# wuer5/OMGSR

Measured on AMD Instinct MI355X. Metric: SR images/sec, higher is better.
Workload: dtype fp16; 1 GPU; OMGSR-S 256->1024, batch=4/GPU, accurate tier (fp32 stream, fp16 MFMA operands + split corrections), tiled VAE 256/64; global_batch=4, latent_tile=64, tile_overlap=32, world_size=1, parallelism=dp1, weights=seeded random, SD2.1-base shapes

## Files before the change

### include/omgsr_hip.h

```cpp
#ifndef OMGSR_HIP_H
#define OMGSR_HIP_H

#include <stdint.h>

#ifdef __cplusplus
extern "C" {
#endif

#define OMGSR_E_BADARG (-1)
#define OMGSR_E_SHAPE (-2)
#define OMGSR_E_ARCH (-3)

#define OMGSR_ACT_NONE 0
#define OMGSR_ACT_SILU 1
#define OMGSR_ACT_GELU_TANH 2
#define OMGSR_ACT_GEGLU 3

#define OMGSR_OUT_BF16 0
#define OMGSR_OUT_F32 1

#define OMGSR_LAYOUT_NHWC 0
#define OMGSR_LAYOUT_T 1

#define OMGSR_EL_16 0
// ... 46 lines not shown
    int32_t mx_scale_w1, mx_scale_a1, mx_scale_w2, mx_scale_a2;
    int32_t out_mx;
    int32_t group_tiles;
    uint32_t* overflow_flag;
    const float* gn_scale_shift;
    int32_t gn_nimg;
    int32_t gn_act;
    int32_t in_el;
    int32_t mx_fmt;
    int32_t mxf8;
    int32_t mxf8_reserved;
    const uint8_t* in_scale;
    const uint8_t* w_scale;
} omgsr_igemm_args;
int32_t omgsr_igemm_gn_fusable(const omgsr_igemm_args* a);
int32_t omgsr_igemm_out_mx6_ok(const omgsr_igemm_args* a);
int omgsr_groupnorm_scale_shift(const float* mean, const float* rstd, const float* gamma, const float* beta, float* out, int32_t nimg, int32_t C,
                                int32_t G, void* stream);
int omgsr_igemm(const omgsr_igemm_args* a, void* stream);
int32_t omgsr_conv_mxfp8_ok(const omgsr_igemm_args* a);
int omgsr_conv_mxfp8(const omgsr_igemm_args* a, void* stream);
int32_t omgsr_conv_mxfp8_multi_ok(const omgsr_igemm_args* args, int32_t count);
int omgsr_conv_mxfp8_multi(const omgsr_igemm_args* args, int32_t count, void* stream);
int omgsr_igemm_multi_plan(omgsr_igemm_args* args, int32_t count);
int omgsr_igemm_multi(const omgsr_igemm_args* args, int32_t count, void* stream);
int omgsr_set_batch_invariant(int on);
int64_t omgsr_igemm_workspace_bytes(const omgsr_igemm_args* a);
int32_t omgsr_igemm_gn_slots(const omgsr_igemm_args* a);
int32_t omgsr_igemm_gn_entries(const omgsr_igemm_args* a);

int omgsr_groupnorm_nchunk(int64_t HW);
int omgsr_groupnorm_stats(const void* x, float* partial, float* mean, float* rstd, float* var_out,
                          int32_t N, int64_t HW, int32_t C, int32_t G, float eps, int32_t x_el, void* stream);
int omgsr_groupnorm_finalize(const float* partial, float* mean, float* rstd, float* var_out, int32_t N,
                             int32_t nslot, int32_t G, int32_t entries, double count, float eps, void* stream);
int omgsr_groupnorm_partial(const void* x, float* partial, int32_t N, int64_t HW, int32_t C, int32_t G, int32_t x_el, void* stream);
#define OMGSR_GN_MAX_GROUPS 8
typedef struct omgsr_gn_merge_args {
    const float* partial[OMGSR_GN_MAX_GROUPS];
    double count[OMGSR_GN_MAX_GROUPS];
    float weight[OMGSR_GN_MAX_GROUPS];
    int32_t tiles[OMGSR_GN_MAX_GROUPS];
    int32_t nslot[OMGSR_GN_MAX_GROUPS];
    int32_t entries[OMGSR_GN_MAX_GROUPS];
    int32_t ngroups;
} omgsr_gn_merge_args;
// ... 122 lines not shown
```

### omgsr_amd/_lib.py

```python
from __future__ import annotations

import ctypes as C
import os

import torch

from .build import lib_path

ABI_VERSION = 22


class OmgsrError(RuntimeError):
    pass


class IgemmArgs(C.Structure):
    _fields_ = [
        ("in_", C.c_void_p), ("weight", C.c_void_p), ("bias", C.c_void_p), ("gate", C.c_void_p),
        ("residual", C.c_void_p), ("out", C.c_void_p),
        ("N", C.c_int32), ("H", C.c_int32), ("W", C.c_int32), ("Cin", C.c_int32),
        ("Cout", C.c_int32), ("Cout_pad", C.c_int32), ("K_pad", C.c_int32),
        ("R", C.c_int32), ("S", C.c_int32), ("stride", C.c_int32), ("pad_top", C.c_int32),
        ("pad_left", C.c_int32), ("upsample", C.c_int32),
        ("Ho", C.c_int32), ("Wo", C.c_int32),
# ... 45 lines not shown

_P, _I, _L, _F = C.c_void_p, C.c_int32, C.c_int64, C.c_float

SIGNATURES = {
    "omgsr_abi_version": (C.c_int, []),
    "omgsr_check_device": (C.c_int, []),
    "omgsr_set_compute_dtype": (C.c_int, [C.c_int]),
    "omgsr_get_compute_dtype": (C.c_int, []),
    "omgsr_error_string": (C.c_char_p, [C.c_int]),
    "omgsr_igemm": (C.c_int, [C.POINTER(IgemmArgs), _P]),
    "omgsr_igemm_multi_plan": (C.c_int, [C.POINTER(IgemmArgs), _I]),
    "omgsr_igemm_multi": (C.c_int, [C.POINTER(IgemmArgs), _I, _P]),
    "omgsr_set_batch_invariant": (C.c_int, [C.c_int]),
    "omgsr_set_attention_defer_max": (C.c_int, [C.c_float]),
    "omgsr_igemm_workspace_bytes": (C.c_int64, [C.POINTER(IgemmArgs)]),
    "omgsr_igemm_gn_slots": (C.c_int32, [C.POINTER(IgemmArgs)]),
    "omgsr_igemm_gn_entries": (C.c_int32, [C.POINTER(IgemmArgs)]),
    "omgsr_igemm_gn_fusable": (C.c_int32, [C.POINTER(IgemmArgs)]),
    "omgsr_igemm_out_mx6_ok": (C.c_int32, [C.POINTER(IgemmArgs)]),
    "omgsr_conv_mxfp8_ok": (C.c_int32, [C.POINTER(IgemmArgs)]),
    "omgsr_conv_mxfp8": (C.c_int, [C.POINTER(IgemmArgs), _P]),
    "omgsr_conv_mxfp8_multi_ok": (C.c_int32, [C.POINTER(IgemmArgs), _I]),
    "omgsr_conv_mxfp8_multi": (C.c_int, [C.POINTER(IgemmArgs), _I, _P]),
    "omgsr_groupnorm_apply_mxfp8": (C.c_int, [_P, _P, _P, _P, _P, _P, _P, _I, _L, _I, _I, _I, _I, _I, _P]),
    "omgsr_groupnorm_apply_mxfp8_multi": (C.c_int, [C.POINTER(GnApplyGroup), _I, _P, _P, _P, _P, _I, _I, _I, _I, _I, _P]),
    "omgsr_groupnorm_scale_shift": (C.c_int, [_P, _P, _P, _P, _P, _I, _I, _I, _P]),
    "omgsr_groupnorm_finalize": (C.c_int, [_P, _P, _P, _P, _I, _I, _I, _I, C.c_double, _F, _P]),
    "omgsr_groupnorm_partial": (C.c_int, [_P, _P, _I, _L, _I, _I, _I, _P]),
    "omgsr_groupnorm_finalize_merged": (C.c_int, [C.POINTER(GnMergeArgs), _P, _P, _P, _I, _I, _F, _P]),
    "omgsr_groupnorm_apply_shared": (C.c_int, [_P, _P, _P, _P, _P, _P, _I, _L, _I, _I, _I, _I, _I, _I, _P, _I, _P, _P]),
    "omgsr_groupnorm_apply_multi": (C.c_int, [C.POINTER(GnApplyGroup), _I, _P, _P, _P, _P, _I, _I, _I, _I, _I, _I, _I, _P, _P]),
    "omgsr_groupnorm_finalize2": (C.c_int, [_P, _I, _I, _P, _I, _I, _P, _P, _P, _I, _I, C.c_double, _F, _P]),
    "omgsr_groupnorm_apply2": (C.c_int, [_P, _P, _I, _P, _P, _P, _P, _P, _I, _L, _I, _I, _I, _I, _P, _I, _P, _P]),
    "omgsr_image_to_model_input": (C.c_int, [_P, _P, _I, _I, _I, _I, _P]),
    "omgsr_colorfix_workspace_bytes": (C.c_int64, [_I, _I, _I, _I]),
    "omgsr_colorfix": (C.c_int, [_P, _I, _P, _P, _P, _I, _I, _I, _I, _I, _P]),
    "omgsr_groupnorm_nchunk": (C.c_int, [_L]),
    "omgsr_groupnorm_stats": (C.c_int, [_P, _P, _P, _P, _P, _I, _L, _I, _I, _F, _I, _P]),
    "omgsr_groupnorm_apply": (C.c_int, [_P, _P, _P, _P, _P, _P, _I, _L, _I, _I, _I, _I, _I, _P, _I, _P, _P]),
    "omgsr_layernorm": (C.c_int, [_P, _P, _P, _P, _L, _I, _F, _I, _I, _P]),
    "omgsr_resize_nearest_exact_nhwc": (C.c_int, [_P, _P, _I, _I, _I, _I, _I, _I, _F, _F, _I, _P]),
    "omgsr_transpose_split": (C.c_int, [_P, _P, _I, _I, _I, _L, _P]),
    "omgsr_to_operand": (C.c_int, [_P, _P, _L, _I, _I, _P, _P]),
    "omgsr_quantize_mxfp8": (C.c_int, [_P, _I, _L, _I, _L, _P, _P, _P]),
    "omgsr_attention": (C.c_int, [C.POINTER(AttnArgs), _P]),
    "omgsr_softmax_rows": (C.c_int, [_P, _P, _L, _I, _I, _P]),
# ... 53 lines not shown
```

### omgsr_amd/build.py

```python
from __future__ import annotations

import hashlib
import os
import shutil
import subprocess
import sys

HERE = os.path.dirname(os.path.abspath(__file__))
CSRC = os.path.join(HERE, "csrc")
LIBDIR = os.path.join(HERE, "lib")
LIBNAME = "libomgsr_hip.so"
SOURCES = ["igemm.hip", "igemm_dma.hip", "igemm_p8.hip", "igemm_gmx.hip", "igemm_halo.hip", "igemm_halo_f16.hip", "igemm_halo_multi.hip", "igemm_halo_mx.hip", "igemm_halo_mx6.hip", "igemm_halo_mx6_flat.hip", "igemm_halo_out6.hip", "igemm_halo_flat.hip", "igemm_halo_gn.hip", "attention.hip", "norm.hip", "elementwise.hip", "colorfix.hip", "preprocess.hip", "mfma_peak.hip", "gemm_mxfp8.hip", "attention_mxfp8.hip", "attention_d512.hip", "conv_mxfp8.hip"]
ARCH = "gfx950"


def lib_path() -> str:
    return os.path.join(LIBDIR, LIBNAME)


def _source_digest() -> str:
    h = hashlib.sha256()
    names = sorted(os.listdir(CSRC)) + [os.path.join("..", "..", "include", "omgsr_hip.h")]
    for n in names:
        p = os.path.join(CSRC, n)
        if os.path.isfile(p):
            h.update(n.encode())
            with open(p, "rb") as f:
                h.update(f.read())
    return h.hexdigest()


def build_library(force: bool = False, verbose: bool = False) -> str:
    hipcc = shutil.which("hipcc") or "/opt/rocm/bin/hipcc"
    os.makedirs(LIBDIR, exist_ok=True)
    out = lib_path()
# ... 127 lines not shown
```

### omgsr_amd/nn.py

```python
from __future__ import annotations

import dataclasses
from typing import Optional

import torch
import torch.nn as nn

from . import ops


def _key(*tensors) -> tuple:
    return ops.mode_key() + tuple((t.data_ptr(), t._version, str(t.device), t.dtype, tuple(t.shape)) if torch.is_tensor(t) else t for t in tensors)


_CACHE_EPOCH = 0


def cache_epoch() -> int:
    return _CACHE_EPOCH


def bump_cache_epoch() -> None:
    global _CACHE_EPOCH
    _CACHE_EPOCH += 1
# ... 79 lines not shown

    def packed_mxfp8(self) -> ops.PackedWeight:
        k = _key(self.weight, self.bias, "mxfp8-conv")
        if getattr(self, "_pk8_key", None) != k:
            bump_cache_epoch()
            _log_rebuild(self._drop_packed_mxfp8)
            self._pk8 = ops.pack_conv_weight_mxfp8(self.weight, self.bias)
            self._pk8_key = k
        return self._pk8

    def _drop_packed_mxfp8(self) -> None:
        self._pk8, self._pk8_key = None, None
        bump_cache_epoch()

    def packed(self) -> ops.PackedWeight:
        sp, wsp, ph = self.in_split(), self.in_wsplit(), self.phase_upsample
        return self._packed(lambda: ops.pack_conv_weight(self.weight, self.bias, cout_multiple=8, split=sp, w_split=wsp, upsample_phases=ph),
                            self.weight, self.bias, sp, wsp, ph)

    def nhwc(self, x, *, pad=None, upsample=False, act=ops.ACT_NONE, residual=None, bias_override=None, stride=None, gn_groups=0,
             out_dtype=ops.OUT_STREAM, out_split=1, gn=None):
        pw = self.packed()
        if bias_override is not None:
            pw = dataclasses.replace(pw, bias=bias_override)
        p = self.padding[0] if pad is None else pad
        if out_dtype == ops.OUT_STREAM and self.out_inner16 and ops.precise():
            out_dtype = ops.OUT_BF16
        fp8_pack = self.packed_mxfp8 if (self.fp8 and gn is not None and bias_override is None) else None
        return ops.conv2d(x, pw, stride=stride or self.stride[0], pad=p, upsample=upsample, act=act, residual=residual,
                          gn_groups=gn_groups, out_dtype=out_dtype, out_split=out_split, gn=gn, fp8_pack=fp8_pack)

    def nhwc_multi(self, xs, *, pad=None, upsample=False, act=ops.ACT_NONE, residuals=None, stride=None, gn_groups=0,
                   out_dtype=ops.OUT_STREAM, out_split=1, gn=None, fp8=False):
        pw = self.packed()
        p = self.padding[0] if pad is None else pad
        if out_dtype == ops.OUT_STREAM and self.out_inner16 and ops.precise():
            out_dtype = ops.OUT_BF16
        fp8_pack = self.packed_mxfp8 if (fp8 and self.fp8 and gn is not None) else None
        return ops.conv2d_multi(list(xs), pw, stride=stride or self.stride[0], pad=p, upsample=upsample, act=act, residuals=residuals,
                                gn_groups=gn_groups, out_dtype=out_dtype, out_split=out_split, gn=gn, fp8_pack=fp8_pack)

    def forward(self, x):
        y = self.nhwc(ops.nchw_to_nhwc(x.contiguous(), ops._round_up(self.in_channels, 8)))
        return ops.nhwc_to_nchw(y, channels=self.out_channels,
                                dtype=ops.io_dtype(x))


# ... 85 lines not shown
```

### omgsr_amd/ops.py

```python
from __future__ import annotations

import ctypes as C
import os
from dataclasses import dataclass
from typing import Optional

import torch

from . import _lib
from ._lib import AttnArgs, IgemmArgs, check

ACT_NONE, ACT_SILU, ACT_GELU_TANH, ACT_GEGLU = 0, 1, 2, 3
OUT_STREAM, OUT_BF16, OUT_F32 = -1, 0, 1
LAYOUT_NHWC, LAYOUT_T = 0, 1
EL_16, EL_F32, EL_SPLIT, EL_MX, EL_MX6, EL_MXFP8 = 0, 1, 2, 3, 4, 5
MX_LO_SHIFT = 11


def _el_of_split(split: int) -> int:
    return {1: EL_16, 2: EL_SPLIT, 3: EL_MX, 4: EL_MX6}[split]


_ACT = torch.bfloat16
_PRECISE = False
# ... 86 lines not shown
_mx_saturated = False


def mx_saturation_seen(reset: bool = True) -> bool:
    global _mx_saturated
    for t in _ovf_words.values():
        if int(t.item()) & 2:
            _mx_saturated = True
            if reset:
                t.bitwise_and_(1)
    seen = _mx_saturated
    if reset:
        _mx_saturated = False
    return seen


_BATCH_INVARIANT = False


def set_batch_invariant(on: bool) -> None:
    global _BATCH_INVARIANT
    check(_lib.load().omgsr_set_batch_invariant(int(bool(on))), "omgsr_set_batch_invariant")
    _BATCH_INVARIANT = bool(on)


STAGE_NONE, STAGE_ENCODE, STAGE_DENOISE, STAGE_DECODE = 0, 1, 2, 3


def timing_stage(stage: int) -> None:
    _lib.load().omgsr_timing_stage(stage)


def compute_dtype_name() -> str:
    return "fp32" if _PRECISE else ("bf16" if _ACT == torch.bfloat16 else "fp16")


def io_dtype(x: torch.Tensor) -> torch.dtype:
    return torch.float32 if x.dtype == torch.float32 else _ACT


def _el(t: torch.Tensor, name: str) -> int:
    if not t.is_cuda:
        raise _lib.OmgsrError(f"{name}: tensor is on {t.device}; the OMGSR HIP path runs on an MI355X only")
    if not t.is_contiguous():
        raise ValueError(f"{name}: must be contiguous")
    if t.dtype == torch.float32:
# ... 33 lines not shown
        ws = torch.empty(need // 4, device=device, dtype=torch.float32)
        a.workspace = ws.data_ptr()
    check(lib.omgsr_igemm(C.byref(a), _stream()), what)



@dataclass
class PackedWeight:
    w: torch.Tensor
    bias: Optional[torch.Tensor]
    cout: int
    cin: int
    R: int
    S: int
    geglu: bool = False
    w_cm: Optional[torch.Tensor] = None
    split: int = 1
    mx: Optional[tuple] = None
    mx_fmt: int = 0
    w_split: int = 1
    in_ld: int = 0
    w_ph: Optional[torch.Tensor] = None
    w_scale: Optional[torch.Tensor] = None

    @property
    def fp8(self) -> bool:
        return self.w_scale is not None

    @property
    def cout_pad(self) -> int:
        return self.w.shape[0]

    @property
    def k_pad(self) -> int:
        return self.w.shape[1]

    @property
    def row_channels(self) -> int:
        return self.in_ld or self.cin


def _segments(w: torch.Tensor, split: int, w_split: int) -> torch.Tensor:
    w_hi = w.to(act_dtype()).float()
    segs = [w_hi] * split
    if w_split == 2:
        segs.append((w - w_hi).to(act_dtype()).float())
# ... 66 lines not shown
    b = None if bias is None else bias.detach().to(device=dev, dtype=torch.float32).contiguous()
    if fmt == 6:
        return PackedWeight(out, b, cout, kslots, R, S, w_cm=w_cm, split=4, w_split=1, in_ld=kslots, w_ph=w_ph, mx=(cin // 32, 127, 127, 127, 127), mx_fmt=6)
    return PackedWeight(out, b, cout, kslots, R, S, w_cm=w_cm, split=3, w_split=1, in_ld=kslots, w_ph=w_ph,
                        mx=(cin // 32, 127 - s1, 127 - MX_LO_SHIFT, 127 - s2, 127))


def _phase_kernels(w: torch.Tensor) -> torch.Tensor:
    rows = {0: ([0], [1, 2]), 1: ([0, 1], [2])}
    w64 = w.double()
    out = []
    for a in (0, 1):
        for b in (0, 1):
            k = torch.zeros((w.shape[0], 2, 2, w.shape[3]), dtype=torch.float64, device=w.device)
            for dy, rs in enumerate(rows[a]):
                for dx, ss in enumerate(rows[b]):
                    for r in rs:
                        for s_ in ss:
                            k[:, dy, dx] += w64[:, r, s_]
            out.append(k.float())
    return torch.stack(out, 0)


def pack_conv_weight(weight: torch.Tensor, bias: Optional[torch.Tensor], device=None, cout_multiple: int = 1,
                     split: int = 1, w_split: int = 1, upsample_phases: bool = False) -> PackedWeight:
    cout, cin, R, S = weight.shape
    dev = device or weight.device
    if cout % cout_multiple:
        extra = _round_up(cout, cout_multiple) - cout
        weight = torch.cat([weight.detach().to(dev), torch.zeros((extra, cin, R, S), device=dev, dtype=weight.dtype)], dim=0)
        if bias is not None:
            bias = torch.cat([bias.detach().to(dev), torch.zeros(extra, device=dev, dtype=bias.dtype)], dim=0)
        cout += extra
    cin8 = _round_up(cin, 8)
    w = _note_weight_range(weight.detach().to(device=dev, dtype=torch.float32)).permute(0, 2, 3, 1)
    if cin8 != cin:
        w = torch.nn.functional.pad(w, (0, cin8 - cin))
    if split in (3, 4):
        if cin8 != cin:
            raise ValueError("the mixed-precision (MX) form needs Cin % 64 == 0")
        return _pack_mx(w, bias if bias is None else bias.detach().to(dev), cout, cin, R, S, dev, upsample_phases, fmt=6 if split == 4 else 8)
    if split not in (1, 2) or w_split not in (1, 2):
        raise ValueError("split / w_split must be 1 or 2")
    if w_split == 2 and bool(torch.equal(w.to(act_dtype()).float(), w)):
        ph_exact = True
        if upsample_phases and R == 3 and S == 3:
            ph0 = _phase_kernels(w)
            ph_exact = bool(torch.equal(ph0.to(act_dtype()).float(), ph0))
        if ph_exact:
            w_split = 1
    in_ld = cin8 * split
    w_raw = w
    w = _segments(w, split, w_split)
    cin8 = w.shape[-1]
    w = w.reshape(cout, R * S * cin8)
    k_pad = _round_up(w.shape[1], 32)
    cout_pad = _round_up(cout, 256 if cout >= 256 else 128)
    out = torch.zeros(cout_pad, k_pad, device=dev, dtype=act_dtype())
    out[:cout, : w.shape[1]] = w.to(act_dtype())
    b = None if bias is None else bias.detach().to(device=dev, dtype=torch.float32).contiguous()
    w_cm = None
    if R == 3 and S == 3 and cin8 % 32 == 0:
        w_cm = out.view(cout_pad, 9, cin8 // 32, 32).permute(2, 1, 0, 3).contiguous()
    w_ph = None
    if upsample_phases and w_cm is not None and in_ld % 32 == 0:
        ph = _segments(_phase_kernels(w_raw), split, w_split).reshape(4, cout, 4 * cin8)
        full = torch.zeros((4, cout_pad, 4 * cin8), device=dev, dtype=act_dtype())
        full[:, :cout] = ph.to(act_dtype())
        w_ph = full.view(4, cout_pad, 4, cin8 // 32, 32).permute(0, 3, 2, 1, 4).contiguous()
    return PackedWeight(out, b, cout, cin8, R, S, w_cm=w_cm, split=split, w_split=w_split, in_ld=in_ld, w_ph=w_ph)


def pack_linear_weight(weight: torch.Tensor, bias: Optional[torch.Tensor], device=None, split: int = 1, w_split: int = 1) -> PackedWeight:
    return pack_conv_weight(weight[:, :, None, None], bias, device, split=split, w_split=w_split)


def pack_geglu_weight(weight: torch.Tensor, bias: Optional[torch.Tensor], device=None, split: int = 1, w_split: int = 1) -> PackedWeight:
    two_inner, cin = weight.shape
    inner = two_inner // 2
    if inner % 32:
        raise ValueError("GEGLU inner dim must be a multiple of 32")
    a, g = weight[:inner], weight[inner:]
    w = torch.stack([a.reshape(inner // 32, 32, cin), g.reshape(inner // 32, 32, cin)], dim=1).reshape(two_inner, cin)
    pw = pack_linear_weight(w, None, device, split=split, w_split=w_split)
    if bias is not None:
        ba, bg = bias[:inner], bias[inner:]
        b = torch.stack([ba.reshape(-1, 32), bg.reshape(-1, 32)], dim=1).reshape(two_inner)
        pw.bias = b.detach().to(device=pw.w.device, dtype=torch.float32).contiguous()
    pw.cout = inner
    pw.geglu = True
    return pw


# ... 201 lines not shown

    def apply(self, x: torch.Tensor, split: int = 1) -> torch.Tensor:
        if split == 5:
            return group_norm_apply_mxfp8(x, self.mean, self.rstd, self.gamma, self.beta, self.groups, self.act)
        if self.mean.shape[0] != x.shape[0]:
            return group_norm_apply_shared(x, self.mean, self.rstd, self.gamma, self.beta, self.groups, self.act, split=split)
        return group_norm_apply(x, self.mean, self.rstd, self.gamma, self.beta, self.groups, self.act, split=split)


def _gn_candidate(x: torch.Tensor, pw: PackedWeight) -> bool:
    return x.dtype == _ACT and pw.split == 1 and pw.w_split == 1 and pw.mx is None and pw.R == 3 and pw.S == 3


def _gn_fusable(a: IgemmArgs, gn: "GnSpec") -> bool:
    return gn.act == ACT_SILU and bool(_lib.load().omgsr_igemm_gn_fusable(C.byref(a)))


def _attach_gn(a: IgemmArgs, gn: "GnSpec", channels: int) -> torch.Tensor:
    t = gn.table(channels)
    a.gn_scale_shift, a.gn_nimg, a.gn_act, a.in_el = t.data_ptr(), t.shape[0], gn.act, EL_16
    return t


def conv2d(x: torch.Tensor, pw: PackedWeight, *, stride: int = 1, pad: tuple[int, int, int, int] | int = 1,
           upsample: bool = False, act: int = ACT_NONE, residual: Optional[torch.Tensor] = None,
           gate: Optional[torch.Tensor] = None, out_dtype: int = OUT_STREAM, alpha: float = 1.0,
           out: Optional[torch.Tensor] = None, gn_groups: int = 0, out_split: int = 1, sample_rows: int = 0,
           gn: Optional["GnSpec"] = None, fp8_pack=None) -> torch.Tensor:
    a = IgemmArgs()
    if gn is not None and not _gn_candidate(x, pw):
        x, gn = gn.apply(x, pw.split), None
    x, out = _conv_args(a, x, pw, stride, pad, upsample, act, residual, gate, out_dtype, alpha, out, out_split, sample_rows)
    if fp8_pack is not None and gn is not None and out_split == 1 and _lib.load().omgsr_conv_mxfp8_ok(C.byref(a)):
        return _conv2d_mxfp8(a, gn.apply(x, 5), fp8_pack(), out, gn_groups)
    if out_split == 4 and not _lib.load().omgsr_igemm_out_mx6_ok(C.byref(a)):
        return to_operand(conv2d(x, pw, stride=stride, pad=pad, upsample=upsample, act=act, residual=residual, gate=gate, out_dtype=OUT_STREAM,
                                 alpha=alpha, sample_rows=sample_rows, gn=gn), 4)
    keep = None
    if gn is not None:
        a.in_el = EL_16
        if _gn_fusable(a, gn):
            keep = _attach_gn(a, gn, x.shape[-1])
        else:
            x = gn.apply(x, pw.split)
            a.in_ = x.data_ptr()
    partial = _conv_gn(a, gn_groups, out_split, x.device)
    _igemm(a, x.device, "omgsr_igemm(conv2d)")
    del keep
    if partial is not None:
        out._omgsr_gn = (partial, gn_groups, out.data_ptr(), out._version)
    return out

# ... 74 lines not shown
        a = arr[i]
        out = _out_tensor((N, H, W), pw8.cout, out_dtype, 1, xq.codes.device)
        residual = None if residuals is None else residuals[i]
        if residual is not None and tuple(residual.shape) != (N, H, W, pw8.cout):
            raise ValueError(f"residual shape {tuple(residual.shape)} != output {(N, H, W, pw8.cout)}")
        _fill_out(a, out, 1, residual, pw8.cout)
        a.N, a.H, a.W, a.Cin, a.Cout = N, H, W, Cin, pw8.cout
        a.R, a.S, a.stride, a.pad_top, a.pad_left, a.upsample = 3, 3, 1, 1, 1, 0
        a.Ho, a.Wo, a.act, a.out_layout = H, W, act, LAYOUT_NHWC
        a.batch, a.alpha, a.sample_rows = 1, 1.0, H * W
        a.overflow_flag = None
        outs.append(out)
    return _conv2d_mxfp8_multi(arr, n, xqs, pw8, outs, gn_groups)


def conv2d_multi(xs, pw: PackedWeight, *, stride: int = 1, pad: tuple[int, int, int, int] | int = 1, upsample: bool = False,
                 act: int = ACT_NONE, residuals=None, out_dtype: int = OUT_STREAM, gn_groups: int = 0, out_split: int = 1,
                 gn: Optional["GnSpec"] = None, fp8_pack=None):
    n = len(xs)
    if n == 1:
        return [conv2d(xs[0], pw, stride=stride, pad=pad, upsample=upsample, act=act, residual=None if residuals is None else residuals[0],
                       out_dtype=out_dtype, gn_groups=gn_groups, out_split=out_split, gn=gn, fp8_pack=fp8_pack)]
    lib = _lib.load()
    if gn is not None and not all(_gn_candidate(x, pw) for x in xs):
        xs, gn = [gn.apply(x, pw.split) for x in xs], None
    arr = (IgemmArgs * n)()
    keep, outs = [], []
    for i in range(n):
        x, out = _conv_args(arr[i], xs[i], pw, stride, pad, upsample, act, None if residuals is None else residuals[i], None, out_dtype, 1.0,
                            None, out_split, 0)
        keep.append(x)
        outs.append(out)
        if gn is not None:
            arr[i].in_el = EL_16
    if fp8_pack is not None and gn is not None and out_split == 1 and lib.omgsr_conv_mxfp8_multi_ok(arr, n):
        xqs = []
        for k in range(0, n, _lib.GN_MAX_GROUPS):
            xqs += group_norm_apply_mxfp8_multi(keep[k:k + _lib.GN_MAX_GROUPS], gn.mean, gn.rstd, gn.gamma, gn.beta, gn.groups, gn.act)
        return _conv2d_mxfp8_multi(arr, n, xqs, fp8_pack(), outs, gn_groups)
    check(lib.omgsr_igemm_multi_plan(arr, n), "omgsr_igemm_multi_plan")
    if out_split == 4 and not all(lib.omgsr_igemm_out_mx6_ok(C.byref(arr[i])) for i in range(n)):
        ys = conv2d_multi(keep, pw, stride=stride, pad=pad, upsample=upsample, act=act, residuals=residuals, out_dtype=OUT_STREAM, gn=gn)
        return [to_operand(y, 4) for y in ys]
    if gn is not None:
        if all(_gn_fusable(arr[i], gn) for i in range(n)):
            for i in range(n):
# ... 793 lines not shown
```

### omgsr_amd/pipelines/vaehook.py

```python
from __future__ import annotations

import math
from typing import Dict, List, Tuple

import torch

from .. import ops


def get_best_tile_size(lowerbound: int, upperbound: int) -> int:
    divider = 32
    while divider >= 2:
        rem = lowerbound % divider
        if rem == 0:
            return lowerbound
        cand = lowerbound - rem + divider
        if cand <= upperbound:
            return cand
        divider //= 2
    return lowerbound


def split_tiles(h: int, w: int, tile_size: int, pad: int, is_decoder: bool) -> Tuple[List[List[int]], List[List[int]]]:
    nh = max(math.ceil((h - 2 * pad) / tile_size), 1)
# ... 71 lines not shown
            return self.net.nhwc(x)
        return self.vae_tile_forward(x)

    def _run(self, seq, groups: Dict[tuple, torch.Tensor], counts: Dict[tuple, int], N: int, fixed=None, record=None):
        res: Dict[tuple, list] = {k: [] for k in groups}
        gi = 0
        pending = None
        for op in seq:
            kind = op[0]
            if kind == "gn":
                norm, act = op[1], op[2]
                G = norm.num_groups
                if fixed is not None:
                    mean, var = fixed[gi]
                    rstd = torch.rsqrt(var + 1e-6)
                else:
                    keys = list(groups)
                    mean, rstd, var = ops.group_norm_stats_merged([groups[k] for k in keys], [counts[k] for k in keys], N, G, 1e-6)
                if record is not None:
                    record.append((mean, var))
                gi += 1
                first = next(iter(groups.values()))
                is_conv3 = getattr(op[3], "kernel_size", None) == (3, 3)
                if is_conv3 and first.dtype != torch.float32:
                    pending = norm.spec_stats(mean, rstd, act)
                    if op[4] is not None:
                        for k in groups:
                            res[k].append(op[4].nhwc(groups[k], pad=0))
                    continue
                keys = list(groups)
                if op[4] is not None:
                    outs = norm.apply_stats_multi([groups[k] for k in keys], mean, rstd, act, split=op[3].in_split(), also_cast=op[4].in_split())
                    for k, (y, xc) in zip(keys, outs):
                        groups[k] = y
                        res[k].append(op[4].nhwc(xc, pad=0))
                else:
                    for k, y in zip(keys, norm.apply_stats_multi([groups[k] for k in keys], mean, rstd, act, split=op[3].in_split())):
                        groups[k] = y
            elif kind == "conv":
                keys = list(groups)
                for k, y in zip(keys, op[1].nhwc_multi([groups[k] for k in keys], gn=pending, fp8=self.fp8_convs, **op[2])):
                    groups[k] = y
                pending = None
            elif kind == "res_push":
                for k in groups:
                    res[k].append(op[1](groups[k]) if op[1] is not None else groups[k])
            elif kind == "conv_res":
# ... 55 lines not shown
```

Measured before the change: 20.90 images/s.

## Add fused GroupNorm+SiLU thin 3x3 conv kernel for few-output-channel convs

Adds a dedicated fp32 direct-convolution HIP kernel for 3x3 convs with at most 8 output channels, such as the VAE encoder's final conv_out. The GroupNorm scale/shift and SiLU are applied while the input tile is staged into LDS, so the separate normalize pass is skipped. It avoids running an implicit GEMM padded to a wide Cout on a very thin output and saves one full activation write plus read. Weights are repacked at load time, and the tiled VAE hook now defers GN into this conv for fp32 inputs. The change adds a new code path with its own multi-tile launcher and tile-height heuristic, and fp32 FMA accumulation order may differ slightly.

Result: no change. 20.95 images/s (median of 5 runs) (+0.2%).

```diff
diff --git a/include/omgsr_hip.h b/include/omgsr_hip.h
--- a/include/omgsr_hip.h
+++ b/include/omgsr_hip.h
@@ -92,6 +92,9 @@
 int omgsr_conv_mxfp8(const omgsr_igemm_args* a, void* stream);
 int32_t omgsr_conv_mxfp8_multi_ok(const omgsr_igemm_args* args, int32_t count);
 int omgsr_conv_mxfp8_multi(const omgsr_igemm_args* args, int32_t count, void* stream);
+int32_t omgsr_conv_thin_ok(const omgsr_igemm_args* a);
+int omgsr_conv_thin(const omgsr_igemm_args* a, void* stream);
+int omgsr_conv_thin_multi(const omgsr_igemm_args* args, int32_t count, void* stream);
 int omgsr_igemm_multi_plan(omgsr_igemm_args* args, int32_t count);
 int omgsr_igemm_multi(const omgsr_igemm_args* args, int32_t count, void* stream);
 int omgsr_set_batch_invariant(int on);
diff --git a/omgsr_amd/_lib.py b/omgsr_amd/_lib.py
--- a/omgsr_amd/_lib.py
+++ b/omgsr_amd/_lib.py
@@ -91,6 +91,9 @@
     "omgsr_conv_mxfp8": (C.c_int, [C.POINTER(IgemmArgs), _P]),
     "omgsr_conv_mxfp8_multi_ok": (C.c_int32, [C.POINTER(IgemmArgs), _I]),
     "omgsr_conv_mxfp8_multi": (C.c_int, [C.POINTER(IgemmArgs), _I, _P]),
+    "omgsr_conv_thin_ok": (C.c_int32, [C.POINTER(IgemmArgs)]),
+    "omgsr_conv_thin": (C.c_int, [C.POINTER(IgemmArgs), _P]),
+    "omgsr_conv_thin_multi": (C.c_int, [C.POINTER(IgemmArgs), _I, _P]),
     "omgsr_groupnorm_apply_mxfp8": (C.c_int, [_P, _P, _P, _P, _P, _P, _P, _I, _L, _I, _I, _I, _I, _I, _P]),
     "omgsr_groupnorm_apply_mxfp8_multi": (C.c_int, [C.POINTER(GnApplyGroup), _I, _P, _P, _P, _P, _I, _I, _I, _I, _I, _P]),
     "omgsr_groupnorm_scale_shift": (C.c_int, [_P, _P, _P, _P, _P, _I, _I, _I, _P]),
diff --git a/omgsr_amd/build.py b/omgsr_amd/build.py
--- a/omgsr_amd/build.py
+++ b/omgsr_amd/build.py
@@ -10,7 +10,7 @@
 CSRC = os.path.join(HERE, "csrc")
 LIBDIR = os.path.join(HERE, "lib")
 LIBNAME = "libomgsr_hip.so"
-SOURCES = ["igemm.hip", "igemm_dma.hip", "igemm_p8.hip", "igemm_gmx.hip", "igemm_halo.hip", "igemm_halo_f16.hip", "igemm_halo_multi.hip", "igemm_halo_mx.hip", "igemm_halo_mx6.hip", "igemm_halo_mx6_flat.hip", "igemm_halo_out6.hip", "igemm_halo_flat.hip", "igemm_halo_gn.hip", "attention.hip", "norm.hip", "elementwise.hip", "colorfix.hip", "preprocess.hip", "mfma_peak.hip", "gemm_mxfp8.hip", "attention_mxfp8.hip", "attention_d512.hip", "conv_mxfp8.hip"]
+SOURCES = ["igemm.hip", "igemm_dma.hip", "igemm_p8.hip", "igemm_gmx.hip", "igemm_halo.hip", "igemm_halo_f16.hip", "igemm_halo_multi.hip", "igemm_halo_mx.hip", "igemm_halo_mx6.hip", "igemm_halo_mx6_flat.hip", "igemm_halo_out6.hip", "igemm_halo_flat.hip", "igemm_halo_gn.hip", "attention.hip", "norm.hip", "elementwise.hip", "colorfix.hip", "preprocess.hip", "mfma_peak.hip", "gemm_mxfp8.hip", "attention_mxfp8.hip", "attention_d512.hip", "conv_mxfp8.hip", "conv_thin.hip"]
 ARCH = "gfx950"
 
 
diff --git a/omgsr_amd/csrc/conv_thin.hip b/omgsr_amd/csrc/conv_thin.hip
--- /dev/null
+++ b/omgsr_amd/csrc/conv_thin.hip
@@ -0,0 +1,206 @@
+#include "common.hip.h"
+#include "../../include/omgsr_hip.h"
+#include "timing.hip.h"
+#include "conv_thin_host.h"
+
+namespace {
+using omgsr::ThinMulti;
+using omgsr::ThinProb;
+
+constexpr int PW = omgsr::THIN_TW + 2;
+constexpr int CK = omgsr::THIN_CK;
+
+template <int TH> struct ThinGeo {
+    static constexpr int NT = TH * 16;
+    static constexpr int NPIX = (TH + 2) * PW;
+    static constexpr int PLANE = NPIX + 2;
+    static constexpr int NLD = (NPIX * (CK / 4) + NT - 1) / NT;
+    static constexpr int LDS_BYTES = (PLANE * CK + 4) * 4;
+    static constexpr __device__ __host__ int plane(const int c) { return c * PLANE + ((c >> 4) << 2); }
+};
+static_assert(ThinGeo<16>::PLANE % 8 == 6 && ThinGeo<8>::PLANE % 8 == 6, "bank layout of the channel planes");
+
+template <int TH, int NC, bool SILU>
+OMGSR_DEVINL void thin_body(const ThinProb p, const float* __restrict__ w, const float* __restrict__ bias, const int bid, float* __restrict__ lds) {
+    using G = ThinGeo<TH>;
+    const int tid = (int)threadIdx.x;
+    const int tpi = p.tx * p.ty;
+    const int n = bid / tpi, trem = bid - n * tpi;
+    const int tyi = trem / p.tx, txi = trem - tyi * p.tx;
+    const int y0 = tyi * TH, x0 = txi * omgsr::THIN_TW;
+    const int Cin = p.Cin;
+    const float* __restrict__ in = p.in;
+
+    const int q = tid & 7;
+    int poff[G::NLD];
+    unsigned inside = 0;
+#pragma unroll
+    for (int i = 0; i < G::NLD; ++i) {
+        const int pix = (i * G::NT + tid) >> 3;
+        const int py = pix / PW, px = pix - py * PW;
+        const int gy = y0 - 1 + py, gx = x0 - 1 + px;
+        const bool ok = pix < G::NPIX && gy >= 0 && gy < p.H && gx >= 0 && gx < p.W;
+        const int cy = gy < 0 ? 0 : (gy >= p.H ? p.H - 1 : gy), cx = gx < 0 ? 0 : (gx >= p.W ? p.W - 1 : gx);
+        poff[i] = (n * p.H + cy) * p.W + cx;
+        inside |= (ok ? 1u : 0u) << i;
+    }
+    const float* __restrict__ tab = p.table ? p.table + (int64_t)(n % p.nimg) * Cin * 2 : nullptr;
+
+    f32x4_t v[G::NLD];
+    f32x4_t t0 = {1.0f, 0.0f, 1.0f, 0.0f}, t1 = {1.0f, 0.0f, 1.0f, 0.0f};
+    auto issue = [&](const int c0) {
+        int cq = c0 + 4 * q;
+        cq = cq > Cin - 4 ? Cin - 4 : cq;
+#pragma unroll
+        for (int i = 0; i < G::NLD; ++i) v[i] = *reinterpret_cast<const f32x4_t*>(in + (int64_t)poff[i] * Cin + cq);
+        if (tab) {
+            t0 = *reinterpret_cast<const f32x4_t*>(tab + 2 * cq);
+            t1 = *reinterpret_cast<const f32x4_t*>(tab + 2 * cq + 4);
+        }
+    };
+
+    const int oy = tid >> 4, ox = (tid & 15) * 2;
+    float acc[2][NC];
+#pragma unroll
+    for (int o = 0; o < NC; ++o) acc[0][o] = acc[1][o] = bias[o];
+
+    issue(0);
+    for (int c0 = 0; c0 < Cin; c0 += CK) {
+#pragma unroll
+        for (int i = 0; i < G::NLD; ++i) {
+            const int pix = (i * G::NT + tid) >> 3;
+            float f[4] = {__builtin_fmaf(v[i][0], t0[0], t0[1]), __builtin_fmaf(v[i][1], t0[2], t0[3]),
+                          __builtin_fmaf(v[i][2], t1[0], t1[1]), __builtin_fmaf(v[i][3], t1[2], t1[3])};
+            const bool ok = (inside >> i) & 1u;
+#pragma unroll
+            for (int j = 0; j < 4; ++j) {
+                if constexpr (SILU) f[j] = silu_f(f[j]);
+                f[j] = ok ? f[j] : 0.0f;
+            }
+            if (pix < G::NPIX) {
+#pragma unroll
+                for (int j = 0; j < 4; ++j) lds[G::plane(4 * q + j) + pix] = f[j];
+            }
+        }
+        __syncthreads();
+        if (c0 + CK < Cin) issue(c0 + CK);
+        int nac = (Cin - c0) >> 3;
+        nac = nac > CK / 8 ? CK / 8 : nac;
+        for (int ac = 0; ac < nac; ++ac) {
+            const float* __restrict__ wc = w + (int64_t)(c0 + ac * 8) * 8;
+            float part[2][NC];
+#pragma unroll
+            for (int o = 0; o < NC; ++o) part[0][o] = part[1][o] = 0.0f;
+#pragma unroll 1
+            for (int r = 0; r < 3; ++r) {
+                float a[8][4];
+#pragma unroll
+                for (int ch = 0; ch < 8; ++ch) {
+                    const float* src = lds + G::plane(ac * 8 + ch) + (oy + r) * PW + ox;
+                    const f32x2_t lo = *reinterpret_cast<const f32x2_t*>(src), hi = *reinterpret_cast<const f32x2_t*>(src + 2);
+                    a[ch][0] = lo[0]; a[ch][1] = lo[1]; a[ch][2] = hi[0]; a[ch][3] = hi[1];
+                }
+#pragma unroll
+                for (int s = 0; s < 3; ++s) {
+                    const float* __restrict__ wt = wc + (int64_t)(r * 3 + s) * Cin * 8;
+#pragma unroll
+                    for (int ch = 0; ch < 8; ++ch) {
+#pragma unroll
+                        for (int o = 0; o < NC; ++o) {
+                            const float wv = wt[ch * 8 + o];
+                            part[0][o] = __builtin_fmaf(a[ch][s], wv, part[0][o]);
+                            part[1][o] = __builtin_fmaf(a[ch][s + 1], wv, part[1][o]);
+                        }
+                    }
+                    __builtin_amdgcn_sched_barrier(0);
+                }
+            }
+#pragma unroll
+            for (int o = 0; o < NC; ++o) { acc[0][o] += part[0][o]; acc[1][o] += part[1][o]; }
+        }
+        __syncthreads();
+    }
+
+    const int y = y0 + oy, x = x0 + ox;
+    if (y < p.H) {
+        float* dst = p.out + ((int64_t)(n * p.H + y) * p.W + x) * 8;
+#pragma unroll
+        for (int e = 0; e < 2; ++e) {
+            if (x + e < p.W) {
+                *reinterpret_cast<f32x4_t*>(dst + 8 * e) = (f32x4_t){acc[e][0], acc[e][1], acc[e][2], acc[e][3]};
+                if constexpr (NC == 8) *reinterpret_cast<f32x4_t*>(dst + 8 * e + 4) = (f32x4_t){acc[e][4], acc[e][5], acc[e][6], acc[e][7]};
+                else *reinterpret_cast<f32x4_t*>(dst + 8 * e + 4) = (f32x4_t){0.0f, 0.0f, 0.0f, 0.0f};
+            }
+        }
+    }
+}
+
+template <int TH, int NC, bool SILU>
+__global__ __launch_bounds__(TH * 16, 2) void gn_conv3x3_thin_kernel(const ThinProb p, const float* __restrict__ w, const float* __restrict__ bias) {
+    extern __shared__ __attribute__((aligned(16))) float thin_lds[];
+    thin_body<TH, NC, SILU>(p, w, bias, (int)blockIdx.x, thin_lds);
+}
+
+template <int TH, int NC, bool SILU>
+__global__ __launch_bounds__(TH * 16, 2) void gn_conv3x3_thin_multi_kernel(const ThinMulti m, const float* __restrict__ w, const float* __restrict__ bias) {
+    extern __shared__ __attribute__((aligned(16))) float thin_lds[];
+    ThinProb p = m.p[0];
+    int first = 0;
+#pragma unroll
+    for (int i = 1; i < omgsr::THIN_MULTI_MAX; ++i)
+        if (i < m.count && (int)blockIdx.x >= m.start[i]) { p = m.p[i]; first = m.start[i]; }
+    thin_body<TH, NC, SILU>(p, w, bias, (int)blockIdx.x - first, thin_lds);
+}
+
+template <int TH, int NC, bool SILU> int thin_launch(const ThinMulti& m, const unsigned blocks, hipStream_t st) {
+    using G = ThinGeo<TH>;
+    static bool attr_set = false;
+    if (!attr_set) {
+        hipError_t e = hipFuncSetAttribute(reinterpret_cast<const void*>(gn_conv3x3_thin_kernel<TH, NC, SILU>), hipFuncAttributeMaxDynamicSharedMemorySize, G::LDS_BYTES);
+        if (e == hipSuccess) e = hipFuncSetAttribute(reinterpret_cast<const void*>(gn_conv3x3_thin_multi_kernel<TH, NC, SILU>), hipFuncAttributeMaxDynamicSharedMemorySize, G::LDS_BYTES);
+        if (e != hipSuccess) return (int)e;
+        attr_set = true;
+    }
+    if (m.count == 1) hipLaunchKernelGGL((gn_conv3x3_thin_kernel<TH, NC, SILU>), dim3(blocks), dim3(G::NT), G::LDS_BYTES, st, m.p[0], m.w, m.bias);
+    else hipLaunchKernelGGL((gn_conv3x3_thin_multi_kernel<TH, NC, SILU>), dim3(blocks), dim3(G::NT), G::LDS_BYTES, st, m, m.w, m.bias);
+    return (int)hipGetLastError();
+}
+
+int thin_run(const omgsr_igemm_args* a, const int count, hipStream_t st) {
+    ThinMulti m;
+    int th = 16;
+    const int64_t blocks = omgsr::thin_plan(a, count, m, th);
+    if (blocks < 0) return (int)blocks;
+    double M = 0.0;
+    for (int i = 0; i < count; ++i) M += (double)a[i].N * a[i].H * a[i].W;
+    omgsr::TimingScope ts(OMGSR_TK_IGEMM, 2.0 * M * 8.0 * 9.0 * a[0].Cin, M * 4.0 * (a[0].Cin + 8.0), st, (long long)M, 8, 9ll * a[0].Cin);
+    if (ts.active) ts.rec.variant = count == 1 ? 23 : 24;
+    const bool silu = a[0].gn_act == OMGSR_ACT_SILU, half = a[0].Cout <= 4;
+    if (th == 16) {
+        if (half) return silu ? thin_launch<16, 4, true>(m, (unsigned)blocks, st) : thin_launch<16, 4, false>(m, (unsigned)blocks, st);
+        return silu ? thin_launch<16, 8, true>(m, (unsigned)blocks, st) : thin_launch<16, 8, false>(m, (unsigned)blocks, st);
+    }
+    if (half) return silu ? thin_launch<8, 4, true>(m, (unsigned)blocks, st) : thin_launch<8, 4, false>(m, (unsigned)blocks, st);
+    return silu ? thin_launch<8, 8, true>(m, (unsigned)blocks, st) : thin_launch<8, 8, false>(m, (unsigned)blocks, st);
+}
+
+}
+
+extern "C" int32_t omgsr_conv_thin_ok(const omgsr_igemm_args* ap) { return (ap && omgsr::thin_ok(*ap)) ? 1 : 0; }
+
+extern "C" int omgsr_conv_thin(const omgsr_igemm_args* ap, void* stream) {
+    if (!ap) return OMGSR_E_BADARG;
+    return thin_run(ap, 1, reinterpret_cast<hipStream_t>(stream));
+}
+
+extern "C" int omgsr_conv_thin_multi(const omgsr_igemm_args* args, int32_t count, void* stream) {
+    if (!args || count < 1) return OMGSR_E_BADARG;
+    for (int i = 0; i < count; ++i)
+        if (!omgsr::thin_ok(args[i]) || !omgsr::thin_same_layer(args[0], args[i])) return OMGSR_E_SHAPE;
+    for (int at = 0; at < count; at += omgsr::THIN_MULTI_MAX) {
+        const int ng = count - at < omgsr::THIN_MULTI_MAX ? count - at : omgsr::THIN_MULTI_MAX;
+        const int rc = thin_run(args + at, ng, reinterpret_cast<hipStream_t>(stream));
+        if (rc != 0) return rc;
+    }
+    return 0;
+}
diff --git a/omgsr_amd/csrc/conv_thin_host.h b/omgsr_amd/csrc/conv_thin_host.h
--- /dev/null
+++ b/omgsr_amd/csrc/conv_thin_host.h
@@ -0,0 +1,88 @@
+#pragma once
+#include <stdint.h>
+#include "../../include/omgsr_hip.h"
+
+namespace omgsr {
+
+constexpr int THIN_TW = 32;
+constexpr int THIN_CK = 32;
+constexpr int THIN_MAX_CIN = 1024;
+constexpr int THIN_MULTI_MAX = 8;
+constexpr int64_t THIN_FILL_BLOCKS = 512;
+
+struct ThinProb {
+    const float* in;
+    const float* table;
+    float* out;
+    int32_t N, H, W, Cin;
+    int32_t nimg;
+    int32_t tx, ty;
+    int32_t reserved;
+};
+
+struct ThinMulti {
+    ThinProb p[THIN_MULTI_MAX];
+    int32_t start[THIN_MULTI_MAX + 1];
+    int32_t count;
+    const float* w;
+    const float* bias;
+};
+
+inline bool thin_ok(const omgsr_igemm_args& a) {
+    if (a.N <= 0 || a.H <= 0 || a.W <= 0 || a.Cin <= 0) return false;
+    if (a.R != 3 || a.S != 3 || a.stride != 1 || a.pad_top != 1 || a.pad_left != 1 || a.upsample != 0 || a.Ho != a.H || a.Wo != a.W) return false;
+    if ((a.Cin % 8) != 0 || a.Cin > THIN_MAX_CIN) return false;
+    if (a.in_el != OMGSR_EL_F32 || a.in_split || a.w_split || (a.in_ld != 0 && a.in_ld != a.Cin)) return false;
+    if (a.Cout < 1 || a.Cout > 8 || (a.out_ld ? a.out_ld : a.Cout) != 8) return false;
+    if (a.residual || a.gate || a.act != OMGSR_ACT_NONE || a.alpha != 1.0f || a.gn_partial) return false;
+    if (a.out_dtype != OMGSR_OUT_F32 || a.out_layout != OMGSR_LAYOUT_NHWC || a.batch != 1) return false;
+    if (a.mx_chunks16 != 0 || a.out_mx != 0 || a.out_lo_off != 0 || a.mxf8 != 0) return false;
+    if (a.gn_act != OMGSR_ACT_NONE && a.gn_act != OMGSR_ACT_SILU) return false;
+    if (a.gn_scale_shift && a.gn_nimg < 1) return false;
+    if (!a.gn_scale_shift && a.gn_act != OMGSR_ACT_NONE) return false;
+    if ((int64_t)a.N * a.H * a.W >= ((int64_t)1 << 31)) return false;
+    return true;
+}
+
+inline int64_t thin_blocks(const omgsr_igemm_args& a, const int th) {
+    return (int64_t)a.N * ((a.H + th - 1) / th) * ((a.W + THIN_TW - 1) / THIN_TW);
+}
+
+inline int thin_tile_rows(const int64_t blocks16) { return blocks16 >= THIN_FILL_BLOCKS ? 16 : 8; }
+
+inline bool thin_same_layer(const omgsr_igemm_args& a, const omgsr_igemm_args& b) {
+    return a.weight_ph == b.weight_ph && a.bias == b.bias && a.Cin == b.Cin && a.Cout == b.Cout && a.gn_act == b.gn_act && (a.gn_scale_shift != nullptr) == (b.gn_scale_shift != nullptr);
+}
+
+inline int64_t thin_plan(const omgsr_igemm_args* a, const int count, ThinMulti& m, int& th) {
+    if (!a || count < 1 || count > THIN_MULTI_MAX) return OMGSR_E_BADARG;
+    int64_t b16 = 0;
+    for (int i = 0; i < count; ++i) {
+        if (!thin_ok(a[i]) || !thin_same_layer(a[0], a[i])) return OMGSR_E_SHAPE;
+        if (!a[i].in || !a[i].out || !a[i].weight_ph || !a[i].bias) return OMGSR_E_BADARG;
+        b16 += thin_blocks(a[i], 16);
+    }
+    th = thin_tile_rows(b16);
+    int64_t at = 0;
+    m = ThinMulti{};
+    m.count = count;
+    m.w = reinterpret_cast<const float*>(a[0].weight_ph);
+    m.bias = a[0].bias;
+    for (int i = 0; i < count; ++i) {
+        ThinProb& p = m.p[i];
+        p.in = reinterpret_cast<const float*>(a[i].in);
+        p.table = a[i].gn_scale_shift;
+        p.out = reinterpret_cast<float*>(a[i].out);
+        p.N = a[i].N; p.H = a[i].H; p.W = a[i].W; p.Cin = a[i].Cin;
+        p.nimg = a[i].gn_scale_shift ? a[i].gn_nimg : 1;
+        p.tx = (a[i].W + THIN_TW - 1) / THIN_TW;
+        p.ty = (a[i].H + th - 1) / th;
+        m.start[i] = (int32_t)at;
+        at += thin_blocks(a[i], th);
+        if (at >= ((int64_t)1 << 31)) return OMGSR_E_SHAPE;
+    }
+    for (int i = count; i <= THIN_MULTI_MAX; ++i) m.start[i] = (int32_t)at;
+    return at;
+}
+
+}
diff --git a/omgsr_amd/nn.py b/omgsr_amd/nn.py
--- a/omgsr_amd/nn.py
+++ b/omgsr_amd/nn.py
@@ -125,7 +125,7 @@
              out_dtype=ops.OUT_STREAM, out_split=1, gn=None):
         pw = self.packed()
         if bias_override is not None:
-            pw = dataclasses.replace(pw, bias=bias_override)
+            pw = dataclasses.replace(pw, bias=bias_override, w_thin=None, b_thin=None)
         p = self.padding[0] if pad is None else pad
         if out_dtype == ops.OUT_STREAM and self.out_inner16 and ops.precise():
             out_dtype = ops.OUT_BF16
diff --git a/omgsr_amd/ops.py b/omgsr_amd/ops.py
--- a/omgsr_amd/ops.py
+++ b/omgsr_amd/ops.py
@@ -132,6 +132,18 @@
     global _BATCH_INVARIANT
     check(_lib.load().omgsr_set_batch_invariant(int(bool(on))), "omgsr_set_batch_invariant")
     _BATCH_INVARIANT = bool(on)
+
+
+_THIN_CONV = os.environ.get("OMGSR_THIN_CONV", "1") != "0"
+
+
+def thin_conv_enabled() -> bool:
+    return _THIN_CONV
+
+
+def set_thin_conv(on: bool) -> None:
+    global _THIN_CONV
+    _THIN_CONV = bool(on)
 
 
 STAGE_NONE, STAGE_ENCODE, STAGE_DENOISE, STAGE_DECODE = 0, 1, 2, 3
@@ -211,6 +223,9 @@
     in_ld: int = 0
     w_ph: Optional[torch.Tensor] = None
     w_scale: Optional[torch.Tensor] = None
+    w_thin: Optional[torch.Tensor] = None
+    b_thin: Optional[torch.Tensor] = None
+    thin_cout: int = 0
 
     @property
     def fp8(self) -> bool:
@@ -323,9 +338,22 @@
     return torch.stack(out, 0)
 
 
+def _pack_thin(w: torch.Tensor, bias: Optional[torch.Tensor], dev):
+    cout, R, S, cin8 = w.shape
+    if R != 3 or S != 3 or cout > 8:
+        return None, None
+    w_thin = torch.zeros((9, cin8, 8), device=dev, dtype=torch.float32)
+    w_thin[:, :, :cout] = w.reshape(cout, 9, cin8).permute(1, 2, 0)
+    b_thin = torch.zeros(8, device=dev, dtype=torch.float32)
+    if bias is not None:
+        b_thin[:cout] = bias.detach().to(device=dev, dtype=torch.float32)
+    return w_thin, b_thin
+
+
 def pack_conv_weight(weight: torch.Tensor, bias: Optional[torch.Tensor], device=None, cout_multiple: int = 1,
                      split: int = 1, w_split: int = 1, upsample_phases: bool = False) -> PackedWeight:
     cout, cin, R, S = weight.shape
+    cout_own = cout
     dev = device or weight.device
     if cout % cout_multiple:
         extra = _round_up(cout, cout_multiple) - cout
@@ -337,10 +365,13 @@
     w = _note_weight_range(weight.detach().to(device=dev, dtype=torch.float32)).permute(0, 2, 3, 1)
     if cin8 != cin:
         w = torch.nn.functional.pad(w, (0, cin8 - cin))
+    w_thin, b_thin = _pack_thin(w, bias, dev)
     if split in (3, 4):
         if cin8 != cin:
             raise ValueError("the mixed-precision (MX) form needs Cin % 64 == 0")
-        return _pack_mx(w, bias if bias is None else bias.detach().to(dev), cout, cin, R, S, dev, upsample_phases, fmt=6 if split == 4 else 8)
+        pw = _pack_mx(w, bias if bias is None else bias.detach().to(dev), cout, cin, R, S, dev, upsample_phases, fmt=6 if split == 4 else 8)
+        pw.w_thin, pw.b_thin, pw.thin_cout = w_thin, b_thin, cout_own
+        return pw
     if split not in (1, 2) or w_split not in (1, 2):
         raise ValueError("split / w_split must be 1 or 2")
     if w_split == 2 and bool(torch.equal(w.to(act_dtype()).float(), w)):
@@ -369,7 +400,7 @@
         full = torch.zeros((4, cout_pad, 4 * cin8), device=dev, dtype=act_dtype())
         full[:, :cout] = ph.to(act_dtype())
         w_ph = full.view(4, cout_pad, 4, cin8 // 32, 32).permute(0, 3, 2, 1, 4).contiguous()
-    return PackedWeight(out, b, cout, cin8, R, S, w_cm=w_cm, split=split, w_split=w_split, in_ld=in_ld, w_ph=w_ph)
+    return PackedWeight(out, b, cout, cin8, R, S, w_cm=w_cm, split=split, w_split=w_split, in_ld=in_ld, w_ph=w_ph, w_thin=w_thin, b_thin=b_thin, thin_cout=cout_own)
 
 
 def pack_linear_weight(weight: torch.Tensor, bias: Optional[torch.Tensor], device=None, split: int = 1, w_split: int = 1) -> PackedWeight:
@@ -617,12 +648,63 @@
     return t
 
 
+def _thin_args(a: IgemmArgs, x: torch.Tensor, pw: PackedWeight, gn: Optional["GnSpec"], out: Optional[torch.Tensor]):
+    N, H, W, Cin = x.shape
+    if out is None:
+        out = torch.empty((N, H, W, 8), device=x.device, dtype=torch.float32)
+    a.in_, a.in_el, a.out = x.data_ptr(), EL_F32, out.data_ptr()
+    a.weight_ph, a.bias = _ptr(pw.w_thin), _ptr(pw.b_thin)
+    a.N, a.H, a.W, a.Cin, a.Ho, a.Wo = N, H, W, Cin, H, W
+    a.Cout, a.out_ld = pw.thin_cout, 8
+    a.R, a.S, a.stride, a.pad_top, a.pad_left, a.upsample = pw.R, pw.S, 1, 1, 1, 0
+    a.act, a.out_dtype, a.out_layout, a.batch, a.alpha = ACT_NONE, OUT_F32, LAYOUT_NHWC, 1, 1.0
+    a.sample_rows = H * W
+    table = None
+    if gn is not None:
+        table = gn.table(Cin)
+        a.gn_scale_shift, a.gn_nimg, a.gn_act = table.data_ptr(), table.shape[0], gn.act
+    return out, table
+
+
+def _thin_candidate(x: torch.Tensor, pw: PackedWeight, stride, pad, upsample, act, residual, gate, out_dtype, alpha, out, gn_groups, out_split) -> bool:
+    return (_THIN_CONV and pw.w_thin is not None and x.dtype == torch.float32 and x.dim() == 4 and x.shape[-1] == pw.w_thin.shape[1] and
+            x.is_contiguous() and stride == 1 and pad in (1, (1, 1, 1, 1)) and not upsample and act == ACT_NONE and residual is None and
+            gate is None and alpha == 1.0 and gn_groups == 0 and out_split == 1 and pw.cout == 8 and
+            (out_dtype == OUT_F32 or (out_dtype == OUT_STREAM and _PRECISE)) and (out is None or out.dtype == torch.float32))
+
+
+def conv2d_thin(x: torch.Tensor, pw: PackedWeight, gn: Optional["GnSpec"] = None, out: Optional[torch.Tensor] = None) -> torch.Tensor:
+    if pw.w_thin is None or x.dtype != torch.float32:
+        raise ValueError("conv2d_thin: an fp32 stream tensor and a packed 3x3 weight with at most 8 output channels (PackedWeight.w_thin)")
+    a = IgemmArgs()
+    out, table = _thin_args(a, x.contiguous(), pw, gn, out)
+    check(_lib.load().omgsr_conv_thin(C.byref(a), _stream()), "omgsr_conv_thin")
+    del table
+    return out
+
+
+def conv2d_thin_multi(xs, pw: PackedWeight, gn: Optional["GnSpec"] = None):
+    xs = [x.contiguous() for x in xs]
+    if not xs or pw.w_thin is None or any(x.dtype != torch.float32 for x in xs):
+        raise ValueError("conv2d_thin_multi: fp32 stream tensors and a packed 3x3 weight with at most 8 output channels (PackedWeight.w_thin)")
+    n = len(xs)
+    arr = (IgemmArgs * n)()
+    keep = [_thin_args(arr[i], xs[i], pw, gn, None) for i in range(n)]
+    check(_lib.load().omgsr_conv_thin_multi(arr, n, _stream()), "omgsr_conv_thin_multi")
+    return [k[0] for k in keep]
+
+
 def conv2d(x: torch.Tensor, pw: PackedWeight, *, stride: int = 1, pad: tuple[int, int, int, int] | int = 1,
            upsample: bool = False, act: int = ACT_NONE, residual: Optional[torch.Tensor] = None,
            gate: Optional[torch.Tensor] = None, out_dtype: int = OUT_STREAM, alpha: float = 1.0,
            out: Optional[torch.Tensor] = None, gn_groups: int = 0, out_split: int = 1, sample_rows: int = 0,
            gn: Optional["GnSpec"] = None, fp8_pack=None) -> torch.Tensor:
     a = IgemmArgs()
+    if gn is not None and _thin_candidate(x, pw, stride, pad, upsample, act, residual, gate, out_dtype, alpha, out, gn_groups, out_split):
+        _thin_args(a, x, pw, None, out)
+        if gn.act in (ACT_NONE, ACT_SILU) and _lib.load().omgsr_conv_thin_ok(C.byref(a)):
+            return conv2d_thin(x, pw, gn, out)
+        a = IgemmArgs()
     if gn is not None and not _gn_candidate(x, pw):
         x, gn = gn.apply(x, pw.split), None
     x, out = _conv_args(a, x, pw, stride, pad, upsample, act, residual, gate, out_dtype, alpha, out, out_split, sample_rows)
@@ -743,6 +825,14 @@
         return [conv2d(xs[0], pw, stride=stride, pad=pad, upsample=upsample, act=act, residual=None if residuals is None else residuals[0],
                        out_dtype=out_dtype, gn_groups=gn_groups, out_split=out_split, gn=gn, fp8_pack=fp8_pack)]
     lib = _lib.load()
+    if gn is not None and gn.act in (ACT_NONE, ACT_SILU) and all(
+            _thin_candidate(x, pw, stride, pad, upsample, act, None if residuals is None else residuals[i], None, out_dtype, 1.0, None, gn_groups,
+                            out_split) for i, x in enumerate(xs)):
+        probe = (IgemmArgs * n)()
+        for i in range(n):
+            _thin_args(probe[i], xs[i], pw, None, xs[i])
+        if all(lib.omgsr_conv_thin_ok(C.byref(probe[i])) for i in range(n)):
+            return conv2d_thin_multi(xs, pw, gn)
     if gn is not None and not all(_gn_candidate(x, pw) for x in xs):
         xs, gn = [gn.apply(x, pw.split) for x in xs], None
     arr = (IgemmArgs * n)()
diff --git a/omgsr_amd/pipelines/vaehook.py b/omgsr_amd/pipelines/vaehook.py
--- a/omgsr_amd/pipelines/vaehook.py
+++ b/omgsr_amd/pipelines/vaehook.py
@@ -117,7 +117,8 @@
                 gi += 1
                 first = next(iter(groups.values()))
                 is_conv3 = getattr(op[3], "kernel_size", None) == (3, 3)
-                if is_conv3 and first.dtype != torch.float32:
+                thin = is_conv3 and first.dtype == torch.float32 and op[3].out_channels <= 8 and op[4] is None and ops.thin_conv_enabled()
+                if thin or (is_conv3 and first.dtype != torch.float32):
                     pending = norm.spec_stats(mean, rstd, act)
                     if op[4] is not None:
                         for k in groups:
```
